# chenxin030/Opengl_Raytracing

Measured on AMD Instinct MI355X. Metric: Mray/s, higher is better.
Workload: dtype f32

## Files before the change

opengl_raytracing_amd/csrc/rt_kernels.hip:

```cpp
#include "rt_device.h"
#include "rt_wire.h"
#include "rt_mesa_math.h"
#include "rt_fastmath.h"

#include <hip/hip_fp16.h>

#define WAVE 64
#define BLOCK_THREADS 256
#define TILE 16

namespace {

struct v3 { float x, y, z; };

__device__ __forceinline__ v3 V3(float x, float y, float z) { v3 r; r.x = x; r.y = y; r.z = z; return r; }
__device__ __forceinline__ v3 V3(float4 q) { return V3(q.x, q.y, q.z); }
__device__ __forceinline__ v3 operator+(v3 a, v3 b) { return V3(a.x + b.x, a.y + b.y, a.z + b.z); }
__device__ __forceinline__ v3 operator-(v3 a, v3 b) { return V3(a.x - b.x, a.y - b.y, a.z - b.z); }
__device__ __forceinline__ v3 operator*(v3 a, v3 b) { return V3(a.x * b.x, a.y * b.y, a.z * b.z); }
__device__ __forceinline__ v3 operator*(v3 a, float s) { return V3(a.x * s, a.y * s, a.z * s); }
__device__ __forceinline__ v3 operator/(v3 a, float s) { return V3(a.x / s, a.y / s, a.z / s); }
__device__ __forceinline__ v3 div3(v3 a, float s) { v3 r; rtf::div3(a.x, a.y, a.z, s, r.x, r.y, r.z); return r; }
__device__ __forceinline__ v3 operator-(v3 a) { return V3(-a.x, -a.y, -a.z); }
__device__ __forceinline__ v3 splat(float s) { return V3(s, s, s); }
// ... 292 lines not shown
        const float *l = (const float *)(lights + (size_t)i * RT_LIGHT_STRIDE);
        int type = ((const int *)l)[0];
        v3 dir = V3(l[8], l[9], l[10]);
        v3 dn = (type == 1) ? normalize(-dir) : normalize(dir);
        float4 *r = lgt + (size_t)i * RT_LGT_F4;
        r[0] = make_float4(l[4], l[5], l[6], __int_as_float(type));
        r[1] = make_float4(dn.x, dn.y, dn.z, l[15]);
        r[2] = make_float4(l[12], l[13], l[14], l[18] * 0.005f);
        r[3] = make_float4(__int_as_float(((const int *)l)[19]),
                           __int_as_float(((const int *)l)[20]),
                           l[21] * 0.1f, 0.0f);
    }
    for (int i = threadIdx.x; i < RT_HALTON_N; i += blockDim.x) {
        h2[i] = halton_eval(i, 2);
        h3[i] = halton_eval(i, 3);
    }
    float4 *tab = (float4 *)(h3 + RT_HALTON_N);
    for (int k = threadIdx.x; k < nLt * RT_PCF_TAB_N; k += blockDim.x) {
        const int li = k / RT_PCF_TAB_N, sidx = k % RT_PCF_TAB_N;
        const float *l = (const float *)(lights + (size_t)li * RT_LIGHT_STRIDE);
        const int type = ((const int *)l)[0];
        float4 t0 = make_float4(0.f, 0.f, 0.f, 0.f), t1 = t0;
        if (type == 1) {
            const v3 lightDir = normalize(-V3(l[8], l[9], l[10]));
            const float filterSize = l[18] * 0.005f;
            const v3 tangent = normalize(cross(lightDir, V3(0.0f, 1.0f, 0.0f)));
            const v3 bitangent = cross(lightDir, tangent);
            const float rx = fract(halton_eval(sidx, 2) + 0.0f), ry = fract(halton_eval(sidx, 3) + 0.0f);
            const v3 jd = (lightDir + (tangent * rx) * filterSize) + (bitangent * ry) * filterSize;
            t0 = make_float4(jd.x, jd.y, jd.z, dot(jd, jd));
            t1 = make_float4(1.0f / jd.x, 1.0f / jd.y, 1.0f / jd.z, 0.0f);
        }
        tab[2 * k] = t0;
        tab[2 * k + 1] = t1;
    }
}

struct LaneLds {
    SceneLds v;
    int nObj, nLt;
    static constexpr bool fastPbr = false;
    __device__ __forceinline__ const float4 *rec(int i) const { return v.hot + i * RT_HOT_F4; }
    __device__ __forceinline__ float4 light(int i, int k) const { return (v.lgt + i * RT_LGT_F4)[k]; }
    __device__ __forceinline__ float halton(int which, int i, int base) const {
        return (i < RT_HALTON_N) ? (which ? v.halton3 : v.halton2)[i] : halton_eval(i, base);
    }
    __device__ __forceinline__ const float4 *lane_hot(int idx) const { return v.hot + idx * RT_HOT_F4; }
    __device__ __forceinline__ const float4 *lane_mat(int idx) const { return v.mat + idx * RT_MAT_F4; }
    __device__ __forceinline__ bool shape(const Ray &r, float a, const float4 *h, float4 h0, float4, float &t) const {
        return shape_test(r, a, h, __float_as_int(h0.w), t);
    }
    __device__ __forceinline__ int closest(const Ray &r, float maxDist, float &tOut) const {
        v3 inv;
        rtf::rcp3(r.d.x, r.d.y, r.d.z, inv.x, inv.y, inv.z);
        float a = dot(r.d, r.d);
        float minT = maxDist;
        int hit = -1;
        for (int i = 0; i < nObj; i++) {
            const float4 *h = rec(i);
            const float4 h0 = h[0], h1 = h[1];
            if (aabb_test(r, inv, h0, h1, maxDist)) {
                float t;
                if (shape_test(r, a, h, __float_as_int(h0.w), t) && t > 0.0f && t < minT) {
                    minT = t;
                    hit = i;
                }
            }
        }
        tOut = minT;
        return hit;
    }
    template <int COUNT>
    __device__ __forceinline__ bool any(const Ray &r, float maxDist, float limit, unsigned &rays) const {
        return lane_any<COUNT>(*this, nObj, r, maxDist, limit, rays);
    }
};

#ifndef RT_V0_WAVES
#define RT_V0_WAVES 0
#endif
#if RT_V0_WAVES > 0
#define RT_V0_BOUNDS __launch_bounds__(BLOCK_THREADS, RT_V0_WAVES)
#else
#define RT_V0_BOUNDS __launch_bounds__(BLOCK_THREADS)
#endif
template <int COUNT>
__global__ RT_V0_BOUNDS void rt_render_kernel(const RtFrame f, const RtDeviceScene dsc,
                                                                  float4 *__restrict__ gColor,
                                                                  float4 *__restrict__ gPosition,
                                                                  uint2 *__restrict__ gNormal,
                                                                  unsigned long long *rayCounter) {
    extern __shared__ float4 lds[];
    const int nF4 = f.nObj * (RT_HOT_F4 + RT_MAT_F4) + f.nLt * RT_LGT_F4 + 2 * (RT_HALTON_N / 4);
    for (int i = threadIdx.x; i < nF4; i += BLOCK_THREADS) lds[i] = dsc.compiled[i];
    __syncthreads();
    LaneLds sc;
    sc.nObj = f.nObj;
    sc.nLt = f.nLt;
    sc.v.hot = lds;
    sc.v.mat = sc.v.hot + f.nObj * RT_HOT_F4;
    sc.v.lgt = sc.v.mat + f.nObj * RT_MAT_F4;
    sc.v.halton2 = (const float *)(sc.v.lgt + f.nLt * RT_LGT_F4);
    sc.v.halton3 = sc.v.halton2 + RT_HALTON_N;

    const int wave = threadIdx.x >> 6, lane = threadIdx.x & 63;
    const int i = blockIdx.x * TILE + (wave & 1) * 8 + (lane & 7);
    const int j = blockIdx.y * TILE + (wave >> 1) * 8 + (lane >> 3);
    unsigned rays = 0;
    if (i < f.p.regionW && j < f.p.regionH) {
    const int gxI = f.p.x0 + i;
    const int ly = f.p.y0 + j;
    const int gyI = (ly / f.p.stripRows) * f.p.stripCycleRows + f.p.stripOffsetRows + ly % f.p.stripRows;
    const size_t outIdx = f.imageStores ? (size_t)gyI * f.p.width + gxI : (size_t)j * f.p.regionW + i;
    if (gxI >= f.p.width || gyI >= f.p.height) {
        if (!f.imageStores) {
            gColor[outIdx] = make_float4(0.0f, 0.0f, 0.0f, 0.0f);
            gPosition[outIdx] = make_float4(0.0f, 0.0f, 0.0f, 0.0f);
            gNormal[outIdx] = make_uint2(0u, 0u);
        }
    } else {
    const unsigned gx = (unsigned)gxI, gy = (unsigned)gyI;

    const float nz = sample_noise(f, dsc.noise, gx, gy);
    const LanePath out = lane_path<COUNT>(sc, f, dsc.sky, camera_ray(f, nz, gxI, gyI), f.p.maxRayDistance, gx, gy, nz, rays);
    const v3 P = out.P, N = out.N;

    gColor[outIdx] = make_float4(out.color.x, out.color.y, out.color.z, 1.0f);
    gPosition[outIdx] = make_float4(P.x, P.y, P.z, 1.0f);
    gNormal[outIdx] = make_uint2(f2h_rtz(N.x) | (f2h_rtz(N.y) << 16), f2h_rtz(N.z) | (0x3c00u << 16));

    }
    }

    if (COUNT) {
        unsigned long long *blockRays = (unsigned long long *)(lds + nF4);
        if (threadIdx.x == 0) *blockRays = 0ull;
        __syncthreads();
        atomicAdd(blockRays, (unsigned long long)rays);
        __syncthreads();
        if (threadIdx.x == 0) atomicAdd(rayCounter, *blockRays);
    }
}

#ifndef RT_FB_ACCUM
#define RT_FB_ACCUM 1
#endif
template <int COUNT, int BT, bool COMPACT, typename PROFILE, int FIRST = 0>
__global__ __launch_bounds__(BT, PROFILE::waves)
void rt_render_packet_kernel(const RtFrame f, const RtDeviceScene dsc, float4 *__restrict__ gColor,
                             float4 *__restrict__ gPosition, uint2 *__restrict__ gNormal,
                             unsigned long long *rayCounter) {
    static_assert(FIRST == 0 || COUNT == 0, "a frame that records or replays first hits has no ray counter");
    static_assert(BT == 64 && COMPACT, "one-wave workgroups, only the AABBs staged in LDS");
    if constexpr (FIRST == 2) {
        const unsigned tile_ = dsc.tileOrder ? dsc.tileOrder[blockIdx.x] : blockIdx.x;
        if (tile_ < gridDim.x) {
            const unsigned tilesX_ = (unsigned)(f.p.regionW + 7) / 8u;
            const long long t0_ = clock64();
            if (pk_replay_settled_tile(f, (int)(tile_ % tilesX_), (int)(tile_ / tilesX_), (const unsigned char *)rayCounter, gColor, gPosition, gNormal)) {
                if (dsc.tileCost && (threadIdx.x & 63) == 0) {
                    const unsigned c_ = (unsigned)(((unsigned long long)(clock64() - t0_)) >> 6);
                    if (RT_FB_ACCUM) atomicAdd(&dsc.tileCost[tile_], c_);
                    else dsc.tileCost[tile_] = c_;
                }
                return;
            }
        }
    }
    extern __shared__ float4 lds[];
    const int nAll = f.nObj * (RT_HOT_F4 + RT_MAT_F4) + f.nLt * RT_LGT_F4 + 2 * (RT_HALTON_N / 4);
    const int nF4 = PROFILE::boundsLds ? f.nObj * 2 : 0;
    for (int i = threadIdx.x; i < nF4; i += BT) lds[i] = dsc.compiled[(i >> 1) * RT_HOT_F4 + (i & 1)];
    __syncthreads();
    SceneLds sc;
    sc.compact = true;
    sc.boundsLds = PROFILE::boundsLds;
    sc.straight = PROFILE::straight;
    sc.split = PROFILE::split;
    sc.hotStride = 2;
    sc.matF4Base = f.nObj * RT_HOT_F4;
    sc.hot = lds;
    sc.mat = sc.hot + f.nObj * RT_HOT_F4;
    sc.lgt = sc.mat + f.nObj * RT_MAT_F4;
    sc.halton2 = (const float *)(sc.lgt + f.nLt * RT_LGT_F4);
    sc.halton3 = sc.halton2 + RT_HALTON_N;
    sc.stats = COUNT ? rayCounter : nullptr;
    sc.global = dsc.compiled;
    sc.lgtF4Base = f.nObj * (RT_HOT_F4 + RT_MAT_F4);
    sc.haltonFloatBase = (sc.lgtF4Base + f.nLt * RT_LGT_F4) * 4;
    sc.park = (float *)(lds + nF4 + 1);
    sc.pcfTabF4 = dsc.noise ? -1 : nAll;
    sc.stab = dsc.shadowTab;

    const int tilesX = (f.p.regionW + 7) / 8;
    const unsigned tile = dsc.tileOrder ? dsc.tileOrder[blockIdx.x] : blockIdx.x;
    if (tile >= gridDim.x) return;
    sc.tileX = (int)(tile % (unsigned)tilesX);
    sc.tileY = (int)(tile / (unsigned)tilesX);
    const long long t0 = clock64();

    unsigned rays = 0;
    if constexpr (FIRST != 0) render_packet<COUNT, BT, PROFILE, FIRST>(f, dsc, sc, gColor, gPosition, gNormal, rays, (uint2 *)rayCounter);
    else render_packet<COUNT, BT, PROFILE>(f, dsc, sc, gColor, gPosition, gNormal, rays);

    if (dsc.tileCost && (threadIdx.x & 63) == 0) {
        const unsigned c = (unsigned)(((unsigned long long)(clock64() - t0)) >> 6);
        if (RT_FB_ACCUM) atomicAdd(&dsc.tileCost[tile], c);
        else dsc.tileCost[tile] = c;
    }

    if (COUNT) {
        unsigned long long *blockRays = (unsigned long long *)(lds + nF4);
        if (threadIdx.x == 0) *blockRays = 0ull;
        __syncthreads();
        atomicAdd(blockRays, (unsigned long long)rays);
        __syncthreads();
        if (threadIdx.x == 0) atomicAdd(rayCounter, *blockRays);
    }
}

__global__ __launch_bounds__(64) void rt_predict_tiles_kernel(const RtFrame f, const RtDeviceScene dsc, int tilesX, int nTiles,
                                                               unsigned *__restrict__ seg, int segStride, unsigned *__restrict__ cursors,
                                                               unsigned *__restrict__ nextCursors, unsigned char *__restrict__ cls) {
    const int lane = threadIdx.x;
    const int tile = blockIdx.x * 64 + lane;
    const bool valid = tile < nTiles;
    if (blockIdx.x == 0 && lane < 32) nextCursors[lane] = 0u;
    extern __shared__ float4 lds[];
    for (int k = lane; k < f.nObj * RT_HOT_F4; k += 64) lds[k] = dsc.compiled[k];
    __syncthreads();
    SceneLds sc;
    sc.hot = lds;
    sc.mat = dsc.compiled + f.nObj * RT_HOT_F4;
    sc.lgt = sc.mat + f.nObj * RT_MAT_F4;
    sc.global = dsc.compiled;
    sc.compact = true;
    sc.matF4Base = f.nObj * RT_HOT_F4;
    sc.lgtF4Base = f.nObj * (RT_HOT_F4 + RT_MAT_F4);
    const int tx = valid ? tile % tilesX : 0, ty = valid ? tile / tilesX : 0;
    const int i = min(tx * 8 + 4, f.p.regionW - 1), j = min(ty * 8 + 4, f.p.regionH - 1);
    const int gxI = f.p.x0 + i, ly = f.p.y0 + j;
    const int gyI = (ly / f.p.stripRows) * f.p.stripCycleRows + f.p.stripOffsetRows + ly % f.p.stripRows;
    float cost = 300.0f;
    bool alive = valid && gxI < f.p.width && gyI < f.p.height;
    const float nz = alive ? sample_noise(f, dsc.noise, (unsigned)gxI, (unsigned)gyI) : 0.0f;
    Ray ray;
    {
        float ux = (((float)gxI + 0.5f) + (nz * 2.0f - 1.0f)) / (float)f.p.width, uy = (((float)gyI + 0.5f) - 1.0f) / (float)f.p.height;
        ux = (ux * 2.0f - 1.0f) * f.sx;
        uy = (uy * 2.0f - 1.0f) * f.sy;
        const v3 cd = V3(f.p.camDir[0], f.p.camDir[1], f.p.camDir[2]), cr = V3(f.p.camRight[0], f.p.camRight[1], f.p.camRight[2]),
                 cu = V3(f.p.camUp[0], f.p.camUp[1], f.p.camUp[2]);
        ray.o = V3(f.p.camPos[0], f.p.camPos[1], f.p.camPos[2]);
        ray.d = normalize((cd + cr * ux) + cu * uy);
    }
    const float travCost = 250.0f + 12.0f * (float)min(f.nObj, 64) + 2.0f * (float)f.nObj;
    const float cand = 1.5f + (float)f.nObj * (1.0f / 28.0f);
    for (int depth = 0; depth < f.p.maxRayDepth; ++depth) {
        if (__builtin_amdgcn_ballot_w64(alive) == 0ull) break;
        float t = f.p.maxRayDistance;
        int idx = -1;
        {
            v3 inv;
            inv.x = __builtin_amdgcn_rcpf(ray.d.x); inv.y = __builtin_amdgcn_rcpf(ray.d.y); inv.z = __builtin_amdgcn_rcpf(ray.d.z);
            const float a = dot(ray.d, ray.d);
            for (int k = 0; k < f.nObj; k++) {
                const float4 *h = lds + k * RT_HOT_F4;
                const float4 h0 = h[0], h1 = h[1];
                if (alive && aabb_test(ray, inv, h0, h1, f.p.maxRayDistance)) {
                    float tt;
                    if (shape_test(ray, a, h, __float_as_int(h0.w), tt) && tt > 0.0f && tt < t) { t = tt; idx = k; }
                }
            }
        }
        if (alive) cost += travCost;
        alive = alive && idx >= 0;
        const int ii = alive ? idx : 0;
        const float4 hb = lds[ii * RT_HOT_F4], h2 = lds[ii * RT_HOT_F4 + 2], h3 = lds[ii * RT_HOT_F4 + 3];
        const float4 m1 = pk_lane_mat(sc, ii, 1), m2 = pk_lane_mat(sc, ii, 2);
        const v3 P = ray.o + ray.d * t;
        const v3 N = (__float_as_int(hb.w) == 0) ? normalize(P - V3(h2)) : V3(h3);
        if (alive) cost += 350.0f;
        for (int li = 0; li < f.nLt; li++) {
            const int lb4 = sc.lgtF4Base + li * RT_LGT_F4;
            const float4 l0 = uni_load4(sc, lb4), l1 = uni_load4(sc, lb4 + 1), l3 = uni_load4(sc, lb4 + 3);
            const int ltype = __float_as_int(l0.w), shadowType = __float_as_int(l3.x), pcf = max(__float_as_int(l3.y), 0);
            v3 lightDir = V3(l1);
            bool lit = alive;
            if (ltype != 1) {
                lightDir = V3(l0) - P;
                lightDir = lightDir * __builtin_amdgcn_rsqf(dot(lightDir, lightDir));
                if (ltype == 2) lit = lit && dot(lightDir, V3(l1)) > 0.0f;
            }
            lit = lit && dot(N, lightDir) > 0.0f;
            if (alive) cost += 330.0f;
            if (lit && (shadowType == 1 || shadowType == 2)) {
                cost += 120.0f + (float)min(pcf, 64) * (50.0f + 70.0f * cand);
                if (shadowType == 2) cost += 16.0f * (60.0f + 25.0f * (float)min(f.nObj, 32));
            }
        }
        if (alive && m2.w > 0.0f) cost += 4.0f * (travCost + 60.0f);
        if (depth + 1 >= f.p.maxRayDepth) break;
        if (alive) {
            const v3 O = P + N * 0.001f;
            if (m1.y > 0.0f) {
                const int dd = depth < RT_MAX_DEPTH ? depth : RT_MAX_DEPTH - 1;
                ray.d = normalize(mix_fast(reflect(ray.d, N), hemisphere_dir(V3(f.hemi[dd][0], f.hemi[dd][1], f.hemi[dd][2]), N), m1.x));
                ray.o = O;
            } else if (m1.w > 0.0f) {
                ray.d = calc_refraction(ray, N, m1.z);
                ray.o = P - N * 0.001f;
            } else {
                ray.d = reflect(ray.d, N);
                ray.o = O;
            }
        }
    }
    cost = (cost == cost) ? fminf(cost, 3.0e38f) : 3.0e38f;
    int c = (int)(4.0f * __log2f(fmaxf(cost, 1.0f))) - 32;
    c = min(max(c, 0), 31);
    {
        const int cl = __shfl_up(c, 1), cr2 = __shfl_down(c, 1);
        const int nb = max((lane & 63) > 0 ? cl : 0, (lane & 63) < 63 ? cr2 : 0);
        c = max(c, nb - 1);
    }
    if (valid && cls) cls[tile] = (unsigned char)c;
    unsigned long long rem = __builtin_amdgcn_ballot_w64(valid);
    while (rem) {
        const int c0 = __builtin_amdgcn_readlane(c, __builtin_ctzll(rem));
        const bool sel = valid && c == c0;
        const unsigned long long mm = __builtin_amdgcn_ballot_w64(sel);
        const int first = __builtin_ctzll(mm);
        unsigned base = 0;
        if (lane == first) base = atomicAdd(&cursors[c0], (unsigned)__builtin_popcountll(mm));
        base = (unsigned)__builtin_amdgcn_readlane((int)base, first);
        if (sel) {
            const unsigned pos = base + (unsigned)__builtin_popcountll(mm & ((1ull << lane) - 1ull));
            if (pos < (unsigned)segStride) seg[(size_t)c0 * segStride + pos] = (unsigned)tile;
        }
        rem &= ~mm;
    }
}

template <typename U>
__global__ void rt_deinterleave_kernel(const U *__restrict__ src, U *__restrict__ dst, int rowUnits,
                                       int height, int stripRows, int stripCount, size_t rankStrideUnits) {
    const size_t total = (size_t)rowUnits * height;
    for (size_t k = (size_t)blockIdx.x * blockDim.x + threadIdx.x; k < total; k += (size_t)gridDim.x * blockDim.x) {
// ... 362 lines not shown
```

opengl_raytracing_amd/csrc/rt_packet.inc:

```
#ifndef RT_PK_LIGHT_SCENE
#define RT_PK_LIGHT_SCENE 32
#endif
#ifndef RT_PK_STRAIGHT
#define RT_PK_STRAIGHT 12
#endif
#ifndef RT_LIGHT_FAST_PBR
#define RT_LIGHT_FAST_PBR 1
#endif
#ifndef RT_HEAVY_FAST_PBR
#define RT_HEAVY_FAST_PBR 1
#endif
#ifndef RT_LIGHT_GROUPN
#define RT_LIGHT_GROUPN 4
#endif
#ifndef RT_HEAVY_GROUPN
#define RT_HEAVY_GROUPN 2
#endif
#ifndef RT_LIGHT_SSS_GROUP
#define RT_LIGHT_SSS_GROUP 4
#endif
#ifndef RT_HEAVY_SSS_GROUP
#define RT_HEAVY_SSS_GROUP 2
#endif
#ifndef RT_PK_BLOCKER_GROUP
// ... 923 lines not shown
            if (tabF4 >= 0 && s < RT_PCF_TAB_N) {
                const float4 t0 = uni_load4(sc, tabF4 + 2 * s), t1 = uni_load4(sc, tabF4 + 2 * s + 1);
                sr[k].d = V3(t0);
                a[k] = t0.w;
                inv[k] = V3(t1);
            } else {
            float rx = fract(pk_halton(sc, 0, s, 2) + nz);
            float ry = fract(pk_halton(sc, 1, s, 3) + 0.0f);
            v3 jd = (lightDir + (tangent * rx) * filterSize) + (bitangent * ry) * filterSize;
            if (ltype != 1) jd = normalize(jd);
            sr[k].d = jd;
            rtf::rcp3(jd.x, jd.y, jd.z, inv[k].x, inv[k].y, inv[k].z);
            a[k] = dot(jd, jd);
            }
        }
        for (int base = 0; base < nObj; base += 64) {
            const int ci = base >> 6;
            unsigned long long m = 0ull;
#pragma unroll
            for (int c = 0; c < CACHE; c++) m = (ci == c) ? cm[c] : m;
            if (NWT == 0 && !cached) {
                float4 bmn = make_float4(0.f, 0.f, 0.f, 0.f), bmx = make_float4(0.f, 0.f, 0.f, 0.f);
                bool bnan = false;
                if (base + lane < nObj) {
                    bmn = pk_bounds(sc, base + lane, 0);
                    bmx = pk_bounds(sc, base + lane, 1);
                    bnan = bounds_nan(bmn, bmx);
                }
                m = light_mask(bmn, bmx, base + lane < nObj, bnan);
                const int ns = pcfSamples - s0 < GROUPN ? pcfSamples - s0 : GROUPN;
                if (base == 0) pk_stat<COUNT>(sc, 1, (unsigned long long)ns);
                pk_stat<COUNT>(sc, 2, (unsigned long long)__builtin_popcountll(m) * (unsigned long long)ns);
                pk_stat<COUNT>(sc, (pk.cull && pk.okx && pk.oky && pk.okz) ? 9 : 10, (unsigned long long)__builtin_popcountll(m) * (unsigned long long)ns);
                pk_stat<COUNT>(sc, 3, 1);
            }
            while (m) {
                bool anyTodo = false;
#pragma unroll
                for (int k = 0; k < GROUPN; k++) anyTodo |= todo[k];
                if (!wave_any(anyTodo)) break;
                const int bit = __builtin_ctzll(m);
                const int i = base + bit;
                m &= m - 1;
                const float4 h0 = uni_load4(sc, i * RT_HOT_F4), h1 = uni_load4(sc, i * RT_HOT_F4 + 1);
                const int type = __float_as_int(h0.w);
#if RT_PK_TIMERS
                pk_stat<COUNT>(sc, 22, 1);
                {
                    bool anyPass = false;
#pragma unroll
                    for (int k = 0; k < GROUPN; k++) anyPass |= todo[k] && aabb_test(sr[k], inv[k], h0, h1, maxDist);
                    if (wave_any(anyPass)) pk_stat<COUNT>(sc, 23, 1);
                    pk_stat<COUNT>(sc, 24, (unsigned long long)__builtin_popcountll(__builtin_amdgcn_ballot_w64(anyPass)));
                }
#endif
#pragma unroll
                for (int k = 0; k < GROUPN; k++) {
                    if (sc.straight & 4) {
                    const bool pass = todo[k] & aabb_test(sr[k], inv[k], h0, h1, maxDist);
                    if (pk_wave_any(pass)) {
                        float t = 0.0f;
                        const bool occ = pk_shape_hit(sc, sr[k], a[k], i, h1.w, type, pass, t) & (t > 0.0f) & (t < limit);
                        todo[k] = todo[k] & !occ;
                    }
                    } else {
                    if (todo[k] && aabb_test(sr[k], inv[k], h0, h1, maxDist)) {
                        float t;
                        if (pk_shape_test(sc, sr[k], a[k], i, h1.w, type, t) && t > 0.0f && t < limit) todo[k] = false;
                    }
                    }
                }
            }
        }
#pragma unroll
        for (int k = 0; k < GROUPN; k++) {
            if (s0 + k < pcfSamples) shadow += (need && !todo[k]) ? 0.0f : 1.0f;
        }
    }
    pk_stat<COUNT>(sc, 14, pk_clock<COUNT>() - tMasks);
    return shadow / (float)pcfSamples;
    } else {
    unsigned occBits = 0;
    const unsigned long long tMasks = pk_clock<COUNT>();
    pk_stat<COUNT>(sc, 13, tMasks - tEnter);
    for (int base = 0; base < nObj; base += 64) {
        float4 bmn = make_float4(0.f, 0.f, 0.f, 0.f), bmx = make_float4(0.f, 0.f, 0.f, 0.f);
        bool bnan = false;
        if (NWT == 0 && base + lane < nObj) {
            bmn = pk_bounds(sc, base + lane, 0);
            bmx = pk_bounds(sc, base + lane, 1);
            bnan = bounds_nan(bmn, bmx);
        }
        unsigned long long mask = 0ull;
        if constexpr (NWT > 0) {
#pragma unroll
            for (int c = 0; c < CACHE; c++) mask = ((base >> 6) == c) ? tm[c] : mask;
        } else {
            mask = light_mask(bmn, bmx, base + lane < nObj, bnan);
        }
        if (NWT == 0)
        pk_stat<COUNT>(sc, 2, (unsigned long long)__builtin_popcountll(mask) * (unsigned long long)pcfSamples);
        pk_stat<COUNT>(sc, (pk.cull && pk.okx && pk.oky && pk.okz) ? 9 : 10, (unsigned long long)__builtin_popcountll(mask) * (unsigned long long)pcfSamples);
        pk_stat<COUNT>(sc, 3, 1);
        if (NWT == 0 && base == 0) pk_stat<COUNT>(sc, 1, (unsigned long long)pcfSamples);
        if (mask == 0ull) continue;
        for (int s = 0; s < pcfSamples; s++) {
            bool todo = need && !((occBits >> (s & 31)) & 1u);
            if (!wave_any(todo)) continue;
            Ray sr; sr.o = origin;
            v3 inv; float a;
            if (tabF4 >= 0 && s < RT_PCF_TAB_N) {
                const float4 t0 = uni_load4(sc, tabF4 + 2 * s), t1 = uni_load4(sc, tabF4 + 2 * s + 1);
                sr.d = V3(t0); a = t0.w; inv = V3(t1);
            } else {
                float rx = fract(pk_halton(sc, 0, s, 2) + nz);
                float ry = fract(pk_halton(sc, 1, s, 3) + 0.0f);
                v3 jd = (lightDir + (tangent * rx) * filterSize) + (bitangent * ry) * filterSize;
                if (ltype != 1) jd = normalize(jd);
                sr.d = jd;
                rtf::rcp3(jd.x, jd.y, jd.z, inv.x, inv.y, inv.z);
                a = dot(jd, jd);
            }
            unsigned long long m = mask;
            while (m) {
                const int bit = __builtin_ctzll(m);
                const int i = base + bit;
                m &= m - 1;
                const float4 h0 = uni_load4(sc, i * RT_HOT_F4), h1 = uni_load4(sc, i * RT_HOT_F4 + 1);
                if (sc.straight & 8) {
                const bool pass = todo & aabb_test(sr, inv, h0, h1, maxDist);
                if (pk_wave_any(pass)) {
                    float t = 0.0f;
                    const bool occ = pk_shape_hit(sc, sr, a, i, h1.w, __float_as_int(h0.w), pass, t) & (t > 0.0f) & (t < limit);
                    todo = todo & !occ;
                }
                } else {
                if (todo && aabb_test(sr, inv, h0, h1, maxDist)) {
                    float t;
                    if (pk_shape_test(sc, sr, a, i, h1.w, __float_as_int(h0.w), t) && t > 0.0f && t < limit) todo = false;
                }
                }
                if (!wave_any(todo)) break;
            }
            if (need && !todo) occBits |= 1u << (s & 31);
        }
    }
    float shadow = 0.0f;
    pk_stat<COUNT>(sc, 14, pk_clock<COUNT>() - tMasks);
    for (int s = 0; s < pcfSamples; s++) shadow += ((occBits >> (s & 31)) & 1u) ? 0.0f : 1.0f;
    return shadow / (float)pcfSamples;
    }
}

__device__ __forceinline__ bool pk_replay_settled_tile(const RtFrame &f, int tileX, int tileY, const unsigned char *records, float4 *gColor,
                                                       float4 *gPosition, uint2 *gNormal) {
    const int tilesX = (f.p.regionW + 7) / 8;
    if (!rt_prefix_flag_settled((unsigned)__builtin_amdgcn_readfirstlane((int)records[rt_first_hit_flags_offset(f.p.regionW, f.p.regionH) + (size_t)(tileY * tilesX + tileX)]))) return false;
    const int ln = threadIdx.x & 63;
    const int i = tileX * 8 + (ln & 7), j = tileY * 8 + (ln >> 3);
    if (i < f.p.regionW && j < f.p.regionH) {
        const int gxI = f.p.x0 + i, ly = f.p.y0 + j;
        const int gyI = (ly / f.p.stripRows) * f.p.stripCycleRows + f.p.stripOffsetRows + ly % f.p.stripRows;
        const size_t at = (size_t)j * f.p.regionW + i;
        const size_t out = f.imageStores ? (size_t)gyI * f.p.width + gxI : at;
        if (gxI < f.p.width && gyI < f.p.height) {
            const float4 *fin = (const float4 *)(records + rt_first_hit_finals_offset(f.p.regionW, f.p.regionH)) + 2 * at;
            const float4 a = fin[0], b = fin[1];
            gColor[out] = make_float4(a.x, a.y, a.z, 1.0f);
            gPosition[out] = make_float4(a.w, b.x, b.y, 1.0f);
            gNormal[out] = make_uint2(__float_as_uint(b.z), __float_as_uint(b.w));
        } else if (!f.imageStores) {
            gColor[out] = make_float4(0.0f, 0.0f, 0.0f, 0.0f);
            gPosition[out] = make_float4(0.0f, 0.0f, 0.0f, 0.0f);
            gNormal[out] = make_uint2(0u, 0u);
        }
    }
    return true;
}

template <int COUNT, int BT, typename PROFILE, int FIRST = 0>
__device__ __forceinline__ void render_packet(const RtFrame &f, const RtDeviceScene &dsc, const SceneLds &sc,
                                              float4 *gColor,
                                              float4 *gPosition, uint2 *gNormal, unsigned &rays, uint2 *firstHit = nullptr) {
    static_assert(BT == 64, "one-wave workgroups: the 8x8 tile and the parking area's stride assume it");
    static_assert(FIRST == 0 || COUNT == 0, "the instrumented builds always trace the whole frame");
    constexpr int GROUPN = PROFILE::groupN;
    const int nObj = f.nObj;
    const float maxDist = f.p.maxRayDistance;
    pk_timers_begin<COUNT>();
    const unsigned long long tWave = pk_clock<COUNT>();

    auto pixel = [&](int &gxI, int &gyI, size_t &outIdx) -> bool {
        const int wave = threadIdx.x >> 6, ln = threadIdx.x & 63;
        const int i = sc.tileX * 8 + (wave & 1) * 8 + (ln & 7);
        const int j = sc.tileY * 8 + (wave >> 1) * 8 + (ln >> 3);
        gxI = f.p.x0 + i;
        const int ly = f.p.y0 + j;
        gyI = (ly / f.p.stripRows) * f.p.stripCycleRows + f.p.stripOffsetRows + ly % f.p.stripRows;
        outIdx = f.imageStores ? (size_t)gyI * f.p.width + gxI : (size_t)j * f.p.regionW + i;
        return i < f.p.regionW && j < f.p.regionH;
    };
    [[maybe_unused]] auto firstIndex = [&]() -> long long {
        const int wave = threadIdx.x >> 6, ln = threadIdx.x & 63;
        const int i = sc.tileX * 8 + (wave & 1) * 8 + (ln & 7);
        const int j = sc.tileY * 8 + (wave >> 1) * 8 + (ln >> 3);
        return (i < f.p.regionW && j < f.p.regionH) ? (long long)j * f.p.regionW + i : -1ll;
    };
    [[maybe_unused]] volatile unsigned *const taintWord = (volatile unsigned *)sc.park - 4;
    [[maybe_unused]] auto records = [&]() -> unsigned char * { return (unsigned char *)((uintptr_t)firstHit & ~RT_FIRST_HIT_SWITCHES); };
    if constexpr (FIRST == 1) *taintWord = 0u;
    int gxI, gyI;
    size_t outIdx;
    const bool inWindow0 = pixel(gxI, gyI, outIdx);
    const bool inImage0 = inWindow0 && gxI < f.p.width && gyI < f.p.height;
    bool alive = inImage0;
    const bool inImage = inImage0;
    const unsigned gx = (unsigned)gxI, gy = (unsigned)gyI;

    const float nz = inImage ? sample_noise(f, dsc.noise, gx, gy) : 0.0f;
    const float jx = nz * 2.0f - 1.0f, jy = 0.0f * 2.0f - 1.0f;
    Ray ray;
    {
        float ux = (((float)gxI + 0.5f) + jx) / (float)f.p.width;
        float uy = (((float)gyI + 0.5f) + jy) / (float)f.p.height;
        ux = ux * 2.0f - 1.0f;
        uy = uy * 2.0f - 1.0f;
        ux *= f.sx;
        uy *= f.sy;
        v3 cd = V3(f.p.camDir[0], f.p.camDir[1], f.p.camDir[2]);
        v3 cr = V3(f.p.camRight[0], f.p.camRight[1], f.p.camRight[2]);
        v3 cu = V3(f.p.camUp[0], f.p.camUp[1], f.p.camUp[2]);
        ray.o = V3(f.p.camPos[0], f.p.camPos[1], f.p.camPos[2]);
        ray.d = normalize((cd + cr * ux) + cu * uy);
    }
    v3 P = V3(0.0f, 0.0f, 0.0f), N = V3(0.0f, 0.0f, 0.0f);
    {
        float *pk_ = sc.park + threadIdx.x;
        pk_[0 * BT] = 0.0f; pk_[1 * BT] = 0.0f; pk_[2 * BT] = 0.0f;
        pk_[3 * BT] = 1.0f; pk_[4 * BT] = 1.0f; pk_[5 * BT] = 1.0f;
        pk_[9 * BT] = 0.0f; pk_[10 * BT] = 0.0f; pk_[11 * BT] = 0.0f;
        pk_[12 * BT] = 0.0f; pk_[13 * BT] = 0.0f; pk_[14 * BT] = 0.0f;
    }

    Box3 rayBox;
    rayBox.lox = rayBox.hix = f.p.camPos[0];
    rayBox.loy = rayBox.hiy = f.p.camPos[1];
    rayBox.loz = rayBox.hiz = f.p.camPos[2];
    bool rayBoxFinite = box_finite(rayBox);

    [[maybe_unused]] auto firstRecordHit = [&](float tHit_, int hit_) {
        const long long at = firstIndex();
        if (at >= 0) {
            const pk_u2 rec = {__float_as_uint(tHit_), (unsigned)hit_};
#if RT_FIRST_HIT_NT
            __builtin_nontemporal_store(rec, (pk_u2 *)records() + at);
#else
            ((pk_u2 *)records())[at] = rec;
#endif
        }
    };
    [[maybe_unused]] auto firstRecordColour = [&]() {
        asm volatile("" ::: "memory");
        const float *pk_ = sc.park + threadIdx.x;
        const long long at = firstIndex();
        if (at >= 0) {
            float *col = (float *)(records() + rt_first_hit_colours_offset(f.p.regionW, f.p.regionH)) + 3 * at;
#pragma unroll
            for (int k = 0; k < 3; k++) {
#if RT_FIRST_HIT_NT
                __builtin_nontemporal_store(pk_[k * BT], col + k);
#else
                col[k] = pk_[k * BT];
#endif
            }
        }
    };

    [[maybe_unused]] auto prefixRecord = [&](int depth_, bool alive_, int idx_) {
        asm volatile("" ::: "memory");
        const float *pk_ = sc.park + threadIdx.x;
        const long long at = firstIndex();
        if (at >= 0) {
            const float *tn = pk_ + (alive_ ? 3 : 12) * BT;
            const pk_u2 w01 = {alive_ ? (unsigned)idx_ : 0xffffffffu, __float_as_uint(pk_[0 * BT])};
            const pk_f4 a = {pk_[10 * BT], pk_[11 * BT], tn[0 * BT], tn[1 * BT]};
            const pk_f4 b = {tn[2 * BT], alive_ ? pk_[6 * BT] : 0.0f, alive_ ? pk_[7 * BT] : 0.0f, alive_ ? pk_[8 * BT] : 0.0f};
            float *col = (float *)(records() + rt_first_hit_colours_offset(f.p.regionW, f.p.regionH)) + 3 * at;
            pk_f4 *fin = (pk_f4 *)(records() + rt_first_hit_finals_offset(f.p.regionW, f.p.regionH)) + 2 * at;
            __builtin_nontemporal_store(w01, (pk_u2 *)records() + at);
            __builtin_nontemporal_store(pk_[1 * BT], col + 0);
            __builtin_nontemporal_store(pk_[2 * BT], col + 1);
            __builtin_nontemporal_store(pk_[9 * BT], col + 2);
            __builtin_nontemporal_store(a, fin);
            __builtin_nontemporal_store(b, fin + 1);
        }
        *taintWord = (unsigned)depth_;
    };
    int depth0 = 0;
    if constexpr (FIRST == 2) {
        const unsigned char *base = (const unsigned char *)firstHit;
        int k = rt_prefix_flag_depth((unsigned)__builtin_amdgcn_readfirstlane(
            (int)base[rt_first_hit_flags_offset(f.p.regionW, f.p.regionH) + (size_t)(sc.tileY * ((f.p.regionW + 7) / 8) + sc.tileX)]));
        if (k > RT_PREFIX_CAP) k = RT_PREFIX_CAP;
        if (k > 0) {
            const long long at = firstIndex();
            float *pk_ = sc.park + threadIdx.x;
            int idx = -1;
            alive = false;
            if (at >= 0) {
                const uint2 w01 = firstHit[at];
                const float *col = (const float *)(base + rt_first_hit_colours_offset(f.p.regionW, f.p.regionH)) + 3 * at;
                const float4 *fin = (const float4 *)(base + rt_first_hit_finals_offset(f.p.regionW, f.p.regionH)) + 2 * at;
                const float c0 = col[0], c1 = col[1], c2 = col[2];
                const float4 a = fin[0], b = fin[1];
                const int hitRec = (int)w01.x;
                idx = (hitRec >= 0 && hitRec < nObj) ? hitRec : -1;
                alive = idx >= 0;
                pk_[0 * BT] = __uint_as_float(w01.y); pk_[1 * BT] = c0; pk_[2 * BT] = c1;
                pk_[9 * BT] = c2; pk_[10 * BT] = a.x; pk_[11 * BT] = a.y;
                float *tn = pk_ + (alive ? 3 : 12) * BT;
                tn[0 * BT] = a.z; tn[1 * BT] = a.w; tn[2 * BT] = b.x;
                if (alive) {
                    ray.d = V3(b.y, b.z, b.w);
                    P = V3(c2, a.x, a.y);
                }
            }
            depth0 = f.p.maxRayDepth;
            if (wave_any(alive) && k + 1 < f.p.maxRayDepth) {
                const int ii = alive ? idx : 0;
                const float4 hb = pk_bounds(sc, ii, 0), h2 = pk_lane_hot(sc, ii, 2), h3 = pk_lane_hot(sc, ii, 3);
                const float4 m0 = pk_lane_mat(sc, ii, 0), m1 = pk_lane_mat(sc, ii, 1);
                const v3 Ns = normalize(P - V3(h2));
                N = (__float_as_int(hb.w) == 0) ? Ns : V3(h3);
                const v3 V = normalize(-ray.d);
                pk_[6 * BT] = ray.d.x; pk_[7 * BT] = ray.d.y; pk_[8 * BT] = ray.d.z;
                if (alive) { pk_[12 * BT] = N.x; pk_[13 * BT] = N.y; pk_[14 * BT] = N.z; }
                pk_[15 * BT] = V.x; pk_[16 * BT] = V.y; pk_[17 * BT] = V.z;
                pk_[18 * BT] = m0.x; pk_[19 * BT] = m0.y; pk_[20 * BT] = m0.z;
                pk_[22 * BT] = m1.x;
                {
                    const int depth = k;
#include "rt_packet_bounce.inc"
                }
                rayBox = wave_box(ray.o, alive);
                rayBoxFinite = box_finite(rayBox);
                depth0 = k + 1;
            } else if (wave_any(alive)) {
                const int ii = alive ? idx : 0;
                const float4 hb = pk_bounds(sc, ii, 0), h2 = pk_lane_hot(sc, ii, 2), h3 = pk_lane_hot(sc, ii, 3);
                const v3 Ns = normalize(P - V3(h2));
                N = (__float_as_int(hb.w) == 0) ? Ns : V3(h3);
                if (alive) { pk_[12 * BT] = N.x; pk_[13 * BT] = N.y; pk_[14 * BT] = N.z; }
            }
        }
    }

    for (int depth = depth0; depth < f.p.maxRayDepth; ++depth) {
        if (!wave_any(alive)) {
            if constexpr (FIRST == 1) { if (depth == 0) { firstRecordHit(maxDist, -1); firstRecordColour(); } }
            break;
        }
        bool replay = false;
        if constexpr (FIRST == 2) replay = depth == 0;
        float t;
        int idx;
        unsigned long long tHit = 0ull;
        if (replay) {
            const long long at = firstIndex();
            uint2 rec = make_uint2(__float_as_uint(maxDist), 0xffffffffu);
            v3 recCol = V3(0.0f, 0.0f, 0.0f);
            if (at >= 0) {
                const float *col = (const float *)((const unsigned char *)firstHit + rt_first_hit_colours_offset(f.p.regionW, f.p.regionH)) + 3 * at;
                rec = firstHit[at];
                recCol = V3(col[0], col[1], col[2]);
            }
            const int hitRec = (int)rec.y;
            idx = (hitRec >= 0 && hitRec < nObj) ? hitRec : -1;
            t = __uint_as_float(rec.x);
            float *pk_ = sc.park + threadIdx.x;
            pk_[0 * BT] = recCol.x; pk_[1 * BT] = recCol.y; pk_[2 * BT] = recCol.z;
        } else {
        const unsigned long long tTrace = pk_clock<COUNT>();
        idx = pk_trace_closest<COUNT>(sc, nObj, ray, alive, rayBox, rayBoxFinite, maxDist, t, rays);
        tHit = pk_clock<COUNT>();
        pk_stat<COUNT>(sc, 12, tHit - tTrace);
        const bool missed = alive && idx < 0;
        if (wave_any(missed && f.p.useSkybox && dsc.sky != nullptr)) {
            if (missed && f.p.useSkybox && dsc.sky) {
                float *pk_ = sc.park + threadIdx.x;
                const v3 fc = V3(pk_[0 * BT], pk_[1 * BT], pk_[2 * BT]), thr = V3(pk_[3 * BT], pk_[4 * BT], pk_[5 * BT]);
                const v3 nf = fc + thr * sample_cube(dsc.sky, f.skySize, ray.d);
                pk_[0 * BT] = nf.x; pk_[1 * BT] = nf.y; pk_[2 * BT] = nf.z;
            }
        }
        }
        alive = alive && idx >= 0;
        if constexpr (FIRST == 1) { if (depth == 0) firstRecordHit(t, alive ? idx : -1); }
        if (!wave_any(alive)) {
            if constexpr (FIRST == 1) { if (depth == 0) firstRecordColour(); }
            break;
        }

        v3 albedo; float metallic, roughness;
        const int ii = alive ? idx : 0;
        {
            if constexpr (PROFILE::hitBatch) {
            const float4 hb = pk_bounds(sc, ii, 0), h2 = pk_lane_hot(sc, ii, 2), h3 = pk_lane_hot(sc, ii, 3);
            const float4 m0 = pk_lane_mat(sc, ii, 0), m1 = pk_lane_mat(sc, ii, 1);
            P = ray.o + ray.d * t;
            const v3 Ns = normalize(P - V3(h2));
            N = (__float_as_int(hb.w) == 0) ? Ns : V3(h3);
            albedo = V3(m0); metallic = m0.w; roughness = m1.x;
            } else {
            if (__float_as_int(pk_bounds(sc, ii, 0).w) == 0) N = normalize((ray.o + ray.d * t) - V3(pk_lane_hot(sc, ii, 2)));
            else N = V3(pk_lane_hot(sc, ii, 3));
            P = ray.o + ray.d * t;
            const float4 m0 = pk_lane_mat(sc, ii, 0), m1 = pk_lane_mat(sc, ii, 1);
            albedo = V3(m0); metallic = m0.w; roughness = m1.x;
            }
        }
        v3 V = normalize(-ray.d);
        const v3 shadowOrigin = P + N * 0.001f;
        Box3 shBox = rayBox;
        if (!replay) shBox = wave_box(shadowOrigin, alive);
        const bool shBoxFinite = box_finite(shBox);

        {
            float *pk_ = sc.park + threadIdx.x;
            pk_[6 * BT] = ray.d.x; pk_[7 * BT] = ray.d.y; pk_[8 * BT] = ray.d.z;
            if (alive) {
                pk_[9 * BT] = P.x; pk_[10 * BT] = P.y; pk_[11 * BT] = P.z;
                pk_[12 * BT] = N.x; pk_[13 * BT] = N.y; pk_[14 * BT] = N.z;
            }
            pk_[15 * BT] = V.x; pk_[16 * BT] = V.y; pk_[17 * BT] = V.z;
            pk_[18 * BT] = albedo.x; pk_[19 * BT] = albedo.y; pk_[20 * BT] = albedo.z;
            pk_[21 * BT] = metallic; pk_[22 * BT] = roughness;
        }
        unsigned long long tAfter = 0ull;
        if (!replay) {
        v3 Lo = V3(0.0f, 0.0f, 0.0f);
        const unsigned long long tLights = pk_clock<COUNT>();
        pk_stat<COUNT>(sc, 29, tLights - tHit);
        for (int li = 0; li < f.nLt; li++) {
            const int lb4 = sc.lgtF4Base + li * RT_LGT_F4;
            const float4 l0 = uni_load4(sc, lb4), l1 = uni_load4(sc, lb4 + 1), l2 = uni_load4(sc, lb4 + 2), l3 = uni_load4(sc, lb4 + 3);
            const int ltype = __builtin_amdgcn_readfirstlane(__float_as_int(l0.w));
            v3 Pl, Nl0;
            {
                asm volatile("" ::: "memory");
                const float *pk_ = sc.park + threadIdx.x;
                Pl = V3(pk_[9 * BT], pk_[10 * BT], pk_[11 * BT]);
                Nl0 = V3(pk_[12 * BT], pk_[13 * BT], pk_[14 * BT]);
            }
            v3 lightDir = V3(0.0f, 0.0f, 0.0f);
            float attenuation = 1.0f, lightDistance = 0.0f;
            if (ltype == 0) {
                lightDir = V3(l0) - Pl;
                lightDistance = length(lightDir);
                attenuation = rtf::rcp(1.0f + 0.1f * lightDistance + 0.01f * lightDistance * lightDistance);
                lightDir = normalize(lightDir);
            } else if (ltype == 1) {
                lightDir = V3(l1);
                lightDistance = 1e6f;
            } else if (ltype == 2) {
                lightDir = V3(l0) - Pl;
                float q = dot(lightDir, lightDir);
                lightDistance = length(lightDir);
                lightDir = normalize(lightDir);
                attenuation = rtf::rcp(fabsf(q));
                float lc = fmaxf(dot(lightDir, V3(l1)), 0.0f);
                attenuation *= lc;
            }
            const int shadowType = __builtin_amdgcn_readfirstlane(__float_as_int(l3.x));
            const int pcfSamples = __builtin_amdgcn_readfirstlane(__float_as_int(l3.y));
            float shadowFactor = 1.0f;
            if (shadowType == 1 || shadowType == 2) {
                float limit = (ltype == 1) ? maxDist : fminf(maxDist, lightDistance);
                if (ltype != 1 && !(lightDistance == lightDistance)) limit = -1.0f;
                const float filterSize = l2.w;
                bool lit = alive;
                if (COUNT != 1 && pcfSamples >= 1) {
                    const v3 rad = (V3(l2) * attenuation) * l1.w;
                    const bool shines = ((rad.x != 0.0f) & (rad.x == rad.x)) | ((rad.y != 0.0f) & (rad.y == rad.y)) |
                                        ((rad.z != 0.0f) & (rad.z == rad.z));
                    lit = alive && shines && (fmaxf(dot(Nl0, normalize(lightDir)), 0.0f) > 0.0f);
                }
                bool needPcf = lit;
                if (shadowType == 2) {
                    const float searchSize = l3.z;
                    bool anyBlocker = false;
                    const unsigned long long tBlk = pk_clock<COUNT>();
                    bool hasBlockerTab = false;
                    if constexpr (PROFILE::blockerTab) hasBlockerTab = sc.stab && __builtin_amdgcn_readfirstlane(__float_as_int(st_hdr4(sc, li, 6).x)) != 0;
                    if (PROFILE::blockerTab && hasBlockerTab) {
                        constexpr int NB = RT_PK_BLOCKER_GROUP;
                        constexpr int BW = PROFILE::tabWords > 0 ? PROFILE::tabWords : 1;
                        unsigned bm[BW];
                        st_lane_mask<BW, true>(sc, li, nObj, shadowOrigin, V3(l0), lightDir, lightDistance, dot(Nl0, Nl0), lit, bm);
                        for (int s = 0; s < 16; s += NB) {
                            const bool search = (COUNT == 1) ? lit : (lit && !anyBlocker);
                            if (!wave_any(search)) break;
                            v3 bd[NB];
#pragma unroll
                            for (int k = 0; k < NB; k++) {
                                const float rr = pk_halton(sc, 1, s + k, 3) * 2.0f - 1.0f;
                                bd[k] = normalize((lightDir + splat(rr * searchSize)) + splat(rr * searchSize));
                            }
                            anyBlocker |= pk_trace_any_group_masked<COUNT, NB, BW>(sc, shadowOrigin, bd, search, bm, maxDist, limit, rays);
                        }
                    } else
                    if constexpr (PROFILE::blockerPairs) {
                    constexpr int NB = RT_PK_BLOCKER_GROUP;
                    for (int s = 0; s < 16; s += NB) {
                        const bool search = (COUNT == 1) ? lit : (lit && !anyBlocker);
                        if (!wave_any(search)) break;
                        v3 bd[NB];
#pragma unroll
                        for (int k = 0; k < NB; k++) {
                            const float rr = pk_halton(sc, 1, s + k, 3) * 2.0f - 1.0f;
                            bd[k] = normalize((lightDir + splat(rr * searchSize)) + splat(rr * searchSize));
                        }
                        anyBlocker |= pk_trace_any_group<COUNT, NB>(sc, nObj, shadowOrigin, bd, search, shBox, shBoxFinite, maxDist, limit, rays);
                    }
                    } else {
                    for (int s = 0; s < 16; s++) {
                        const bool search = (COUNT == 1) ? lit : (lit && !anyBlocker);
                        if (!wave_any(search)) break;
                        float rr = pk_halton(sc, 1, s, 3) * 2.0f - 1.0f;
                        v3 sd = (lightDir + splat(rr * searchSize)) + splat(rr * searchSize);
                        Ray sr; sr.o = shadowOrigin; sr.d = normalize(sd);
                        anyBlocker |= pk_trace_any<COUNT>(sc, nObj, sr, search, shBox, shBoxFinite, maxDist, limit, rays);
                    }
                    }
// ... 153 lines not shown
```

Before: 287,600.

## Issue replay record loads early and overlap them with LDS bounds staging

In the first-hit replay kernel variant, the tile flag, first-hit record, colour and the first chunk of AABB bounds are now loaded in a single up-front request, before the settled-tile check. Unsettled tiles then park all replay state into LDS together with the bounds staging, behind one barrier. Later replay code reads the parked values instead of issuing dependent global loads. This is meant to overlap global memory latency and remove the serial flag-then-record load chain. In exchange, settled tiles now perform some loads they do not use, and the park layout adds more LDS slots.

```diff
diff --git a/opengl_raytracing_amd/csrc/rt_kernels.hip b/opengl_raytracing_amd/csrc/rt_kernels.hip
--- a/opengl_raytracing_amd/csrc/rt_kernels.hip
+++ b/opengl_raytracing_amd/csrc/rt_kernels.hip
@@ -468,26 +468,35 @@
                              unsigned long long *rayCounter) {
     static_assert(FIRST == 0 || COUNT == 0, "a frame that records or replays first hits has no ray counter");
     static_assert(BT == 64 && COMPACT, "one-wave workgroups, only the AABBs staged in LDS");
+    extern __shared__ float4 lds[];
+    [[maybe_unused]] unsigned tileReplay = 0u;
     if constexpr (FIRST == 2) {
         const unsigned tile_ = dsc.tileOrder ? dsc.tileOrder[blockIdx.x] : blockIdx.x;
-        if (tile_ < gridDim.x) {
-            const unsigned tilesX_ = (unsigned)(f.p.regionW + 7) / 8u;
-            const long long t0_ = clock64();
-            if (pk_replay_settled_tile(f, (int)(tile_ % tilesX_), (int)(tile_ / tilesX_), (const unsigned char *)rayCounter, gColor, gPosition, gNormal)) {
-                if (dsc.tileCost && (threadIdx.x & 63) == 0) {
-                    const unsigned c_ = (unsigned)(((unsigned long long)(clock64() - t0_)) >> 6);
-                    if (RT_FB_ACCUM) atomicAdd(&dsc.tileCost[tile_], c_);
-                    else dsc.tileCost[tile_] = c_;
-                }
-                return;
+        if (tile_ >= gridDim.x) return;
+        tileReplay = tile_;
+        const unsigned tilesX_ = (unsigned)(f.p.regionW + 7) / 8u;
+        const int tileX_ = (int)(tile_ % tilesX_), tileY_ = (int)(tile_ / tilesX_);
+        const long long t0_ = clock64();
+        PkReplayLoads ld_;
+        pk_replay_request<BT, PROFILE::boundsLds>(f, dsc, tileX_, tileY_, (const unsigned char *)rayCounter, ld_);
+        const unsigned flag_ = (unsigned)__builtin_amdgcn_readfirstlane((int)ld_.flag);
+        if (rt_prefix_flag_settled(flag_)) {
+            pk_replay_settled_tile(f, tileX_, tileY_, (const unsigned char *)rayCounter, gColor, gPosition, gNormal);
+            if (dsc.tileCost && (threadIdx.x & 63) == 0) {
+                const unsigned c_ = (unsigned)(((unsigned long long)(clock64() - t0_)) >> 6);
+                if (RT_FB_ACCUM) atomicAdd(&dsc.tileCost[tile_], c_);
+                else dsc.tileCost[tile_] = c_;
             }
-        }
-    }
-    extern __shared__ float4 lds[];
+            return;
+        }
+        pk_replay_park<BT, PROFILE::boundsLds>(f, dsc, tileX_, tileY_, flag_, (const unsigned char *)rayCounter, lds, ld_);
+    }
     const int nAll = f.nObj * (RT_HOT_F4 + RT_MAT_F4) + f.nLt * RT_LGT_F4 + 2 * (RT_HALTON_N / 4);
     const int nF4 = PROFILE::boundsLds ? f.nObj * 2 : 0;
-    for (int i = threadIdx.x; i < nF4; i += BT) lds[i] = dsc.compiled[(i >> 1) * RT_HOT_F4 + (i & 1)];
-    __syncthreads();
+    if constexpr (FIRST != 2) {
+        for (int i = threadIdx.x; i < nF4; i += BT) lds[i] = dsc.compiled[(i >> 1) * RT_HOT_F4 + (i & 1)];
+        __syncthreads();
+    }
     SceneLds sc;
     sc.compact = true;
     sc.boundsLds = PROFILE::boundsLds;
@@ -509,7 +518,7 @@
     sc.stab = dsc.shadowTab;
 
     const int tilesX = (f.p.regionW + 7) / 8;
-    const unsigned tile = dsc.tileOrder ? dsc.tileOrder[blockIdx.x] : blockIdx.x;
+    const unsigned tile = FIRST == 2 ? tileReplay : dsc.tileOrder ? dsc.tileOrder[blockIdx.x] : blockIdx.x;
     if (tile >= gridDim.x) return;
     sc.tileX = (int)(tile % (unsigned)tilesX);
     sc.tileY = (int)(tile / (unsigned)tilesX);
diff --git a/opengl_raytracing_amd/csrc/rt_packet.inc b/opengl_raytracing_amd/csrc/rt_packet.inc
--- a/opengl_raytracing_amd/csrc/rt_packet.inc
+++ b/opengl_raytracing_amd/csrc/rt_packet.inc
@@ -1099,10 +1099,8 @@
     }
 }
 
-__device__ __forceinline__ bool pk_replay_settled_tile(const RtFrame &f, int tileX, int tileY, const unsigned char *records, float4 *gColor,
+__device__ __forceinline__ void pk_replay_settled_tile(const RtFrame &f, int tileX, int tileY, const unsigned char *records, float4 *gColor,
                                                        float4 *gPosition, uint2 *gNormal) {
-    const int tilesX = (f.p.regionW + 7) / 8;
-    if (!rt_prefix_flag_settled((unsigned)__builtin_amdgcn_readfirstlane((int)records[rt_first_hit_flags_offset(f.p.regionW, f.p.regionH) + (size_t)(tileY * tilesX + tileX)]))) return false;
     const int ln = threadIdx.x & 63;
     const int i = tileX * 8 + (ln & 7), j = tileY * 8 + (ln >> 3);
     if (i < f.p.regionW && j < f.p.regionH) {
@@ -1122,7 +1120,71 @@
             gNormal[out] = make_uint2(0u, 0u);
         }
     }
-    return true;
+}
+
+constexpr int PK_PARK_REC_T = 15, PK_PARK_REC_HIT = 16, PK_PARK_REC_K = 17;
+
+struct PkReplayLoads {
+    unsigned flag;
+    uint2 w01;
+    float c0, c1, c2;
+    float4 bounds;
+};
+template <int BT, bool BOUNDS_LDS>
+__device__ __forceinline__ void pk_replay_request(const RtFrame &f, const RtDeviceScene &dsc, int tileX, int tileY, const unsigned char *records,
+                                                  PkReplayLoads &ld) {
+    const int tilesX = (f.p.regionW + 7) / 8;
+    ld.flag = records[rt_first_hit_flags_offset(f.p.regionW, f.p.regionH) + (size_t)(tileY * tilesX + tileX)];
+    ld.bounds = make_float4(0.0f, 0.0f, 0.0f, 0.0f);
+    if (BOUNDS_LDS && (int)threadIdx.x < f.nObj * 2) ld.bounds = dsc.compiled[(threadIdx.x >> 1) * RT_HOT_F4 + (threadIdx.x & 1)];
+    const int ln = threadIdx.x & 63;
+    const int i = tileX * 8 + (ln & 7), j = tileY * 8 + (ln >> 3);
+    ld.w01 = make_uint2(0u, 0u);
+    ld.c0 = ld.c1 = ld.c2 = 0.0f;
+    if (i < f.p.regionW && j < f.p.regionH) {
+        const size_t at = (size_t)j * f.p.regionW + i;
+        const float *col = (const float *)(records + rt_first_hit_colours_offset(f.p.regionW, f.p.regionH)) + 3 * at;
+        ld.w01 = ((const uint2 *)records)[at];
+        ld.c0 = col[0]; ld.c1 = col[1]; ld.c2 = col[2];
+    }
+}
+template <int BT, bool BOUNDS_LDS>
+__device__ __forceinline__ void pk_replay_park(const RtFrame &f, const RtDeviceScene &dsc, int tileX, int tileY, unsigned flag,
+                                               const unsigned char *records, float4 *lds, const PkReplayLoads &ld) {
+    const int nF4 = BOUNDS_LDS ? f.nObj * 2 : 0;
+    float *pk_ = (float *)(lds + nF4 + 1) + threadIdx.x;
+    int k = rt_prefix_flag_depth(flag);
+    if (k > RT_PREFIX_CAP) k = RT_PREFIX_CAP;
+    const int ln = threadIdx.x & 63;
+    const int i = tileX * 8 + (ln & 7), j = tileY * 8 + (ln >> 3);
+    const bool inWindow = i < f.p.regionW && j < f.p.regionH;
+    float4 a = make_float4(0.0f, 0.0f, 0.0f, 0.0f), b = make_float4(0.0f, 0.0f, 0.0f, 0.0f);
+    if (k > 0 && inWindow) {
+        const float4 *fin = (const float4 *)(records + rt_first_hit_finals_offset(f.p.regionW, f.p.regionH)) + 2 * ((size_t)j * f.p.regionW + i);
+        a = fin[0]; b = fin[1];
+    }
+    if ((int)threadIdx.x < nF4) lds[threadIdx.x] = ld.bounds;
+    for (int s = threadIdx.x + BT; s < nF4; s += BT) lds[s] = dsc.compiled[(s >> 1) * RT_HOT_F4 + (s & 1)];
+    if (k > 0) {
+        const int hitRec = inWindow ? (int)ld.w01.x : -1;
+        const int hit = (hitRec >= 0 && hitRec < f.nObj) ? hitRec : -1;
+        const bool alive = hit >= 0;
+        pk_[0 * BT] = __uint_as_float(ld.w01.y); pk_[1 * BT] = ld.c0; pk_[2 * BT] = ld.c1;
+        pk_[3 * BT] = alive ? a.z : 1.0f; pk_[4 * BT] = alive ? a.w : 1.0f; pk_[5 * BT] = alive ? b.x : 1.0f;
+        pk_[6 * BT] = b.y; pk_[7 * BT] = b.z; pk_[8 * BT] = b.w;
+        pk_[9 * BT] = ld.c2; pk_[10 * BT] = a.x; pk_[11 * BT] = a.y;
+        pk_[12 * BT] = alive ? 0.0f : a.z; pk_[13 * BT] = alive ? 0.0f : a.w; pk_[14 * BT] = alive ? 0.0f : b.x;
+        pk_[PK_PARK_REC_HIT * BT] = __int_as_float(hit);
+    } else {
+        pk_[0 * BT] = ld.c0; pk_[1 * BT] = ld.c1; pk_[2 * BT] = ld.c2;
+        pk_[3 * BT] = 1.0f; pk_[4 * BT] = 1.0f; pk_[5 * BT] = 1.0f;
+        pk_[9 * BT] = 0.0f; pk_[10 * BT] = 0.0f; pk_[11 * BT] = 0.0f;
+        pk_[12 * BT] = 0.0f; pk_[13 * BT] = 0.0f; pk_[14 * BT] = 0.0f;
+        pk_[PK_PARK_REC_T * BT] = inWindow ? __uint_as_float(ld.w01.x) : f.p.maxRayDistance;
+        pk_[PK_PARK_REC_HIT * BT] = inWindow ? __uint_as_float(ld.w01.y) : __int_as_float(-1);
+    }
+    pk_[PK_PARK_REC_K * BT] = __int_as_float(k);
+    __syncthreads();
 }
 
 template <int COUNT, int BT, typename PROFILE, int FIRST = 0>
@@ -1181,7 +1243,7 @@
         ray.d = normalize((cd + cr * ux) + cu * uy);
     }
     v3 P = V3(0.0f, 0.0f, 0.0f), N = V3(0.0f, 0.0f, 0.0f);
-    {
+    if constexpr (FIRST != 2) {
         float *pk_ = sc.park + threadIdx.x;
         pk_[0 * BT] = 0.0f; pk_[1 * BT] = 0.0f; pk_[2 * BT] = 0.0f;
         pk_[3 * BT] = 1.0f; pk_[4 * BT] = 1.0f; pk_[5 * BT] = 1.0f;
@@ -1245,32 +1307,14 @@
     };
     int depth0 = 0;
     if constexpr (FIRST == 2) {
-        const unsigned char *base = (const unsigned char *)firstHit;
-        int k = rt_prefix_flag_depth((unsigned)__builtin_amdgcn_readfirstlane(
-            (int)base[rt_first_hit_flags_offset(f.p.regionW, f.p.regionH) + (size_t)(sc.tileY * ((f.p.regionW + 7) / 8) + sc.tileX)]));
-        if (k > RT_PREFIX_CAP) k = RT_PREFIX_CAP;
+        float *pk_ = sc.park + threadIdx.x;
+        const int k = __builtin_amdgcn_readfirstlane(__float_as_int(pk_[PK_PARK_REC_K * BT]));
         if (k > 0) {
-            const long long at = firstIndex();
-            float *pk_ = sc.park + threadIdx.x;
-            int idx = -1;
-            alive = false;
-            if (at >= 0) {
-                const uint2 w01 = firstHit[at];
-                const float *col = (const float *)(base + rt_first_hit_colours_offset(f.p.regionW, f.p.regionH)) + 3 * at;
-                const float4 *fin = (const float4 *)(base + rt_first_hit_finals_offset(f.p.regionW, f.p.regionH)) + 2 * at;
-                const float c0 = col[0], c1 = col[1], c2 = col[2];
-                const float4 a = fin[0], b = fin[1];
-                const int hitRec = (int)w01.x;
-                idx = (hitRec >= 0 && hitRec < nObj) ? hitRec : -1;
-                alive = idx >= 0;
-                pk_[0 * BT] = __uint_as_float(w01.y); pk_[1 * BT] = c0; pk_[2 * BT] = c1;
-                pk_[9 * BT] = c2; pk_[10 * BT] = a.x; pk_[11 * BT] = a.y;
-                float *tn = pk_ + (alive ? 3 : 12) * BT;
-                tn[0 * BT] = a.z; tn[1 * BT] = a.w; tn[2 * BT] = b.x;
-                if (alive) {
-                    ray.d = V3(b.y, b.z, b.w);
-                    P = V3(c2, a.x, a.y);
-                }
+            const int idx = __float_as_int(pk_[PK_PARK_REC_HIT * BT]);
+            alive = idx >= 0;
+            if (alive) {
+                ray.d = V3(pk_[6 * BT], pk_[7 * BT], pk_[8 * BT]);
+                P = V3(pk_[9 * BT], pk_[10 * BT], pk_[11 * BT]);
             }
             depth0 = f.p.maxRayDepth;
             if (wave_any(alive) && k + 1 < f.p.maxRayDepth) {
@@ -1313,19 +1357,10 @@
         int idx;
         unsigned long long tHit = 0ull;
         if (replay) {
-            const long long at = firstIndex();
-            uint2 rec = make_uint2(__float_as_uint(maxDist), 0xffffffffu);
-            v3 recCol = V3(0.0f, 0.0f, 0.0f);
-            if (at >= 0) {
-                const float *col = (const float *)((const unsigned char *)firstHit + rt_first_hit_colours_offset(f.p.regionW, f.p.regionH)) + 3 * at;
-                rec = firstHit[at];
-                recCol = V3(col[0], col[1], col[2]);
-            }
-            const int hitRec = (int)rec.y;
+            const float *pk_ = sc.park + threadIdx.x;
+            const int hitRec = __float_as_int(pk_[PK_PARK_REC_HIT * BT]);
             idx = (hitRec >= 0 && hitRec < nObj) ? hitRec : -1;
-            t = __uint_as_float(rec.x);
-            float *pk_ = sc.park + threadIdx.x;
-            pk_[0 * BT] = recCol.x; pk_[1 * BT] = recCol.y; pk_[2 * BT] = recCol.z;
+            t = pk_[PK_PARK_REC_T * BT];
         } else {
         const unsigned long long tTrace = pk_clock<COUNT>();
         idx = pk_trace_closest<COUNT>(sc, nObj, ray, alive, rayBox, rayBoxFinite, maxDist, t, rays);
```

Measured after the change: 292,700 (median of 6 runs). +1.8%, better.
